# AndrewSigorskih/fastq-dupaway

Measured on AMD Instinct MI355X. Metric: Mreads/s dedup, 150 bp SE FASTQ (device phase: sequences resident in HBM), higher is better.
Workload: dtype u8

## Files before the change

fastq-dupaway_amd/csrc/fqd_engine.hip:

```cpp
#include <hip/hip_runtime.h>

#include <algorithm>
#include <chrono>
#include <cstdio>
#include <cstdlib>
#include <cstring>
#include <string>
#include <vector>

#include "fqd_internal.hpp"
#include "fqd_kernels.hpp"
#include "fqd_table_geometry.hpp"

using namespace fqd;

namespace {

thread_local std::string g_create_error;

struct DevBuf {
    void*  p = nullptr;
    size_t cap = 0;
    template <class T> T* as() const { return static_cast<T*>(p); }
};
// ... 282 lines not shown
    uint64_t* err = e->d_state;
    if (c.staged) {
        const uint32_t per_tile = e->S == 2 ? c.R / 2 : c.R;
        const uint32_t grid = uint32_t(std::min<uint64_t>((n + per_tile - 1) / per_tile, uint64_t(e->n_cu) * blocks_per_cu));
        static const size_t extra_lds = [] { const char* v = std::getenv("FQD_ENC_EXTRA_LDS"); return v ? size_t(std::max(0, std::atoi(v))) : size_t(0); }();
        const size_t lds = size_t(c.tile0) + c.tile1 + extra_lds;
        const uint32_t rw = ks.W0 + ks.lead;
        const uint32_t magic = rw > 1 ? uint32_t(((1ull << 32) + rw - 1) / rw) : 0xFFFFFFFFu;
        if (e->S == 1) {
            static const bool wide_out = [] { const char* v = std::getenv("FQD_ENC_STREAMOUT"); return !(v && v[0] == '0'); }();
            const bool pow2_rows = wide_out && rw >= 2 && (rw & (rw - 1)) == 0 && (reinterpret_cast<uintptr_t>(ks.keys) & 15u) == 0;
            const uint32_t magic1 = (c.lds_out && pow2_rows) ? 0u : magic;
            auto launch = [&](auto kernel) {
                hipLaunchKernelGGL(kernel, dim3(grid), dim3(c.R), lds, stream, sv[0], n, first_idx, ks, hash_out, err, magic1, h1);
            };
            if (c.lds_out) launch(encode_staged_kernel<true>); else launch(encode_staged_kernel<false>);
        } else {
            const uint32_t split = ks.lead + seg_words(seg[0].uniform_len);
            static const bool wide_out = [] { const char* v = std::getenv("FQD_ENC_STREAMOUT"); return !(v && v[0] == '0'); }();
            const bool pow2_rows = wide_out && rw >= 2 && (rw & (rw - 1)) == 0 && (split & 1u) == 0 && (reinterpret_cast<uintptr_t>(ks.keys) & 15u) == 0;
            const uint32_t magic2 = (c.lds_out && pow2_rows) ? 0u : magic;
            auto launch = [&](auto kernel) {
                hipLaunchKernelGGL(kernel, dim3(grid), dim3(c.R), lds, stream,
                                   sv[0], sv[1], n, first_idx, ks, hash_out, err, c.tile0, magic2, h1);
            };
            if (c.lds_out) launch(encode_staged_pe_kernel<true>); else launch(encode_staged_pe_kernel<false>);
        }
    } else if (!(e->flags & FQD_FLAG_NO_STAGE) && sv[0].offsets && (e->S == 1 || sv[1].offsets)) {
        const uint32_t R = 128, span_cap = e->S == 2 ? 24u * 1024u : 48u * 1024u;
        const uint32_t grid = uint32_t(std::min<uint64_t>((n + R - 1) / R, uint64_t(e->n_cu) * blocks_per_cu));
        if (e->S == 1)
            hipLaunchKernelGGL(encode_span_kernel<1>, dim3(grid), dim3(R), span_cap, stream,
                               sv[0], sv[1], n, first_idx, ks, hash_out, err, span_cap, h1);
        else
            hipLaunchKernelGGL(encode_span_kernel<2>, dim3(grid), dim3(R), 2 * span_cap, stream,
                               sv[0], sv[1], n, first_idx, ks, hash_out, err, span_cap, h1);
    } else {
        const uint32_t grid = uint32_t(std::min<uint64_t>(grid_for(e, n), uint64_t(e->n_cu) * blocks_per_cu));
        if (e->S == 1)
            hipLaunchKernelGGL(encode_general_kernel<1>, dim3(grid), dim3(kBlock), 0, stream,
                               sv[0], sv[1], n, first_idx, ks, hash_out, err, h1);
        else
            hipLaunchKernelGGL(encode_general_kernel<2>, dim3(grid), dim3(kBlock), 0, stream,
                               sv[0], sv[1], n, first_idx, ks, hash_out, err, h1);
    }
    HIP_TRY(e, hipGetLastError());
    return FQD_OK;
}

int launch_insert(fqd_engine* e, const KeyStore& ks, const uint64_t* hashes, uint32_t hash_stride,
                  uint64_t n, uint64_t first_idx, uint8_t* keep, bool preset_keep = true, uint32_t blocks_per_cu = 8,
                  uint32_t* first = nullptr)
{
    if (e->table_stale) {
        Bracket br(e, K_OTHER, 0);
        HIP_TRY(e, hipMemsetAsync(e->table.p, 0xFF, e->slots * sizeof(uint64_t), e->stream));
        e->table_stale = false;
    }
    e->table_clear = false;
    if (preset_keep) {
        Bracket br(e, K_OTHER, 0);
        HIP_TRY(e, hipMemsetAsync(keep, 1, n, e->stream));
    }
    Bracket br(e, K_INSERT, n);
    const uint32_t grid = uint32_t(std::min<uint64_t>(grid_for(e, n), uint64_t(e->n_cu) * blocks_per_cu));
    hipLaunchKernelGGL(insert_kernel, dim3(grid), dim3(kBlock), 0, e->stream,
                       e->table.as<uint64_t>(), e->slots - 1, (1ull << e->seg_bits) - 1, ks, hashes, hash_stride, n,
                       Verdicts{keep, first, uint32_t(first_idx)}, e->tag_mask,
                       reinterpret_cast<unsigned long long*>(e->d_state + 1));
    HIP_TRY(e, hipGetLastError());
    return FQD_OK;
}

bool bulk_applies(const fqd_engine* e, uint64_t n)
{
    if (n < e->bulk_min || e->slots < (1ull << 13)) return false;
    const bool empty = e->n_records == 0;
    static const uint64_t ratio = [] { const char* v = std::getenv("FQD_BULK_RATIO"); const long x = v ? std::atol(v) : 12; return uint64_t(x > 0 ? x : 12); }();
    return empty || n * ratio >= e->slots;
}

struct BulkPlan {
    bool ok = false;
    BulkGeom g{0, 0, 0, 0, 0};
    uint32_t nd1 = 0, n_buckets = 0;
    uint32_t *hist1 = nullptr, *start1 = nullptr, *cursor1 = nullptr, *tile_start1 = nullptr;
    uint32_t *hist2 = nullptr, *start2 = nullptr, *cursor2 = nullptr;
    uint64_t *recA = nullptr, *recB = nullptr;
    uint8_t *digit2 = nullptr;
    uint32_t *heavy_count = nullptr, *heavy_list = nullptr;
};

int bulk_plan(fqd_engine* e, uint64_t n, BulkPlan& p)
{
    uint32_t t = 0; while ((1ull << t) < e->slots) ++t;
    const uint32_t nb_bits = t - e->seg_bits;
    p.ok = false;
    if (nb_bits > 17 || nb_bits == 0) return FQD_OK;
    p.g.slot_mask = e->slots - 1; p.g.seg_bits = e->seg_bits; p.g.tag_mask = e->tag_mask;
    fqdgeom::table_digits(t, e->seg_bits, p.g.bits1, p.g.bits2);
    p.nd1 = 1u << p.g.bits1; p.n_buckets = 1u << nb_bits;
    int rc;
    const size_t rec_bytes = ((n * sizeof(uint64_t)) + 255) & ~size_t(255);
    const size_t d2_bytes = p.g.bits2 ? ((n * sizeof(uint8_t)) + 255) & ~size_t(255) : 0;
    if ((rc = reserve(e, e->bulk_recs, rec_bytes * (p.g.bits2 ? 2 : 1) + d2_bytes))) return rc;
    const size_t meta_words = 1100 + 4 * size_t(p.n_buckets) + 16;
    if ((rc = reserve(e, e->bulk_meta, meta_words * sizeof(uint32_t)))) return rc;
    uint32_t* m = e->bulk_meta.as<uint32_t>();
    p.hist1 = m; p.start1 = m + 256; p.cursor1 = m + 520; p.tile_start1 = m + 780;
    p.hist2 = m + 1100; p.start2 = p.hist2 + p.n_buckets; p.cursor2 = p.start2 + p.n_buckets + 4;
    p.heavy_count = m + 1090;
    p.heavy_list = p.cursor2 + p.n_buckets + 4;
    p.recA = e->bulk_recs.as<uint64_t>();
    p.recB = reinterpret_cast<uint64_t*>(e->bulk_recs.as<char>() + rec_bytes);
    p.digit2 = p.g.bits2 ? reinterpret_cast<uint8_t*>(e->bulk_recs.as<char>() + 2 * rec_bytes) : nullptr;
    {
        Bracket br(e, K_OTHER, 0);
        HIP_TRY(e, hipMemsetAsync(m, 0, meta_words * sizeof(uint32_t), e->stream));
    }
    p.ok = true;
    return FQD_OK;
}

int launch_bulk_insert(fqd_engine* e, const KeyStore& ks, const uint64_t* hashes, uint32_t hash_stride,
                       uint64_t n, uint64_t first_idx, uint8_t* keep, const BulkPlan& p, bool hist1_done,
                       uint32_t* first = nullptr, bool last_batch = false)
{
    const Verdicts verdicts{keep, first, uint32_t(first_idx)};
    const BulkGeom g = p.g;
    const uint32_t nd1 = p.nd1, n_buckets = p.n_buckets;
    uint32_t *hist1 = p.hist1, *start1 = p.start1, *cursor1 = p.cursor1, *tile_start1 = p.tile_start1;
    uint32_t *hist2 = p.hist2, *start2 = p.start2, *cursor2 = p.cursor2;
    uint64_t *recA = p.recA, *recB = p.recB;
    const bool fresh = e->n_records == 0 || e->table_clear || e->table_stale;
    {
        Bracket br(e, K_OTHER, 0);
        HIP_TRY(e, hipMemsetAsync(keep, 1, n, e->stream));
    }
    const uint64_t* final_recs = recA; const uint32_t* bstart = start1;
    {
    Bracket part_br(e, K_PARTITION, n);
    uint32_t part_per_cu = 2u;
    if (const char* v = std::getenv("FQD_PART_BLOCKS_PER_CU")) part_per_cu = uint32_t(std::min(16, std::max(1, std::atoi(v))));
    const uint32_t part_grid = uint32_t(std::min<uint64_t>((n + kPartTile - 1) / kPartTile, uint64_t(e->n_cu) * part_per_cu));
    if (!hist1_done)
        hipLaunchKernelGGL(bulk_hist1_kernel, dim3(part_grid), dim3(kPartThreads), 0, e->stream, hashes, hash_stride, n, g, hist1);
    hipLaunchKernelGGL(bulk_scan256_kernel, dim3(1), dim3(320), 0, e->stream,
                       static_cast<const uint32_t*>(hist1), nd1, start1, cursor1, tile_start1);
    hipLaunchKernelGGL(bulk_scatter_kernel<1>, dim3(part_grid), dim3(kPartThreads), 0, e->stream,
                       hashes, hash_stride, uint32_t(first_idx), static_cast<const uint64_t*>(nullptr), n, g,
                       static_cast<const uint32_t*>(start1), static_cast<const uint32_t*>(tile_start1), cursor1, recA, g.bits2 > 8 ? static_cast<uint8_t*>(nullptr) : p.digit2);
    if (g.bits2) {
        const uint32_t grid2 = uint32_t(std::min<uint64_t>((n + kPartTile - 1) / kPartTile + nd1, uint64_t(e->n_cu) * part_per_cu));
        const uint32_t hgrid = uint32_t(std::min<uint64_t>((n + kPartTile - 1) / kPartTile + nd1, uint64_t(e->n_cu) * 2u));
        if (g.bits2 > 8)
            hipLaunchKernelGGL(bulk_hist2_kernel<true>, dim3(hgrid), dim3(kPartThreads), 0, e->stream,
                               static_cast<const uint8_t*>(nullptr), static_cast<const uint64_t*>(recA), g, static_cast<const uint32_t*>(start1),
                               static_cast<const uint32_t*>(tile_start1), hist2);
        else
            hipLaunchKernelGGL(bulk_hist2_kernel<false>, dim3(hgrid), dim3(kPartThreads), 0, e->stream,
                               static_cast<const uint8_t*>(p.digit2), static_cast<const uint64_t*>(nullptr), g, static_cast<const uint32_t*>(start1),
                               static_cast<const uint32_t*>(tile_start1), hist2);
        hipLaunchKernelGGL(bulk_scan_buckets_kernel, dim3(nd1), dim3(512), 0, e->stream,
                           static_cast<const uint32_t*>(hist2), g.bits2, static_cast<const uint32_t*>(start1), nd1, start2, cursor2);
        hipLaunchKernelGGL(bulk_scatter_kernel<2>, dim3(grid2), dim3(kPartThreads), 0, e->stream,
                           static_cast<const uint64_t*>(nullptr), 0u, 0u, static_cast<const uint64_t*>(recA), n, g,
                           static_cast<const uint32_t*>(start1), static_cast<const uint32_t*>(tile_start1), cursor2, recB,
                           static_cast<uint8_t*>(nullptr));
        final_recs = recB; bstart = start2;
    }
    }
    Bracket br(e, K_DEDUP, n);
    const size_t lds = ((size_t(1) << e->seg_bits) + kDedupChunk + 2) * sizeof(uint64_t);
    uint32_t dthreads = 512;
    if (const char* v = std::getenv("FQD_DEDUP_THREADS")) dthreads = uint32_t(std::min(1024, std::max(64, std::atoi(v))));
    const uint32_t dgrid = std::min<uint32_t>(n_buckets, uint32_t(e->n_cu) * uint32_t(std::max<size_t>(1, (160 * 1024) / lds)));
    unsigned long long* counters = reinterpret_cast<unsigned long long*>(e->d_state + 1);
    uint32_t heavy_above = 4u << e->seg_bits;
    if (const char* v = std::getenv("FQD_HEAVY_ABOVE")) heavy_above = uint32_t(std::max(0, std::atoi(v)));
    static const bool force_write_back = [] { const char* v = std::getenv("FQD_FINAL_WRITE_BACK"); return v && v[0] == '1'; }();
    const uint32_t write_back = (last_batch && !force_write_back) ? 0u : 1u;
    auto launch_dedup = [&](auto kernel) -> int {
        if (lds > 64 * 1024) HIP_TRY(e, hipFuncSetAttribute(reinterpret_cast<const void*>(kernel), hipFuncAttributeMaxDynamicSharedMemorySize, int(lds)));
        hipLaunchKernelGGL(kernel, dim3(dgrid), dim3(dthreads), lds, e->stream,
                           final_recs, bstart, n_buckets, e->table.as<uint64_t>(), e->seg_bits, g.seg_bits + g.bits2, ks, verdicts, counters,
                           heavy_above, p.heavy_count, p.heavy_list, write_back);
        return FQD_OK;
    };
    int drc;
    int vl = 0;
    if (!ks.koff && ks.lead == 0 && ks.stride == ks.W0 && (ks.W0 & 1u) == 0) vl = ks.W0 <= 8 ? 4 : (ks.W0 <= 16 ? 8 : 0);
    if (const char* v = std::getenv("FQD_DEDUP_VL")) { if (std::atoi(v) == 0) vl = 0; }
    if (ks.koff)      drc = fresh ? launch_dedup(bucket_dedup_kernel<true, true, 0>) : launch_dedup(bucket_dedup_kernel<false, true, 0>);
    else if (vl == 4) drc = fresh ? launch_dedup(bucket_dedup_kernel<true, false, 4>) : launch_dedup(bucket_dedup_kernel<false, false, 4>);
    else if (vl == 8) drc = fresh ? launch_dedup(bucket_dedup_kernel<true, false, 8>) : launch_dedup(bucket_dedup_kernel<false, false, 8>);
    else              drc = fresh ? launch_dedup(bucket_dedup_kernel<true, false, 0>) : launch_dedup(bucket_dedup_kernel<false, false, 0>);
    if (drc) return drc;
    hipLaunchKernelGGL(heavy_bucket_insert_kernel, dim3(grid_for(e, n)), dim3(kBlock), 0, e->stream,
                       final_recs, bstart, g, e->table.as<uint64_t>(), ks, verdicts, counters,
                       static_cast<const uint32_t*>(p.heavy_count), static_cast<const uint32_t*>(p.heavy_list));
    HIP_TRY(e, hipGetLastError());
    e->table_clear = false; e->table_stale = !write_back;
    return FQD_OK;
}

int check_state(fqd_engine* e)
{
    HIP_TRY(e, hipMemcpyAsync(e->h_state, e->d_state, 5 * sizeof(uint64_t), hipMemcpyDeviceToHost, e->stream));
    HIP_TRY(e, hipStreamSynchronize(e->stream));
    if (e->flags & FQD_FLAG_PROFILE) drain_profile(e);
    if (e->h_state[2] != 0)
        return e->fail(FQD_ERR_HIP, "internal: hash set overflowed its table");
    if (e->h_state[4] != 0)
        return e->fail(FQD_ERR_ARG, "fqd_encode_padded: a read is longer than the key width the caller set (max_len0 / max_len1)");
    if (e->h_state[0] != kNoError) {
        const uint64_t w = e->h_state[0];
        e->has_bad = true;
        e->bad_record = w >> 32; e->bad_seg = uint32_t((w >> 31) & 1u);
        e->bad_pos = uint32_t((w >> 8) & 0x7FFFFFu); e->bad_byte = uint8_t(w & 0xFFu);
        char buf[160];
        std::snprintf(buf, sizeof buf, "unknown character in DNA sequence: byte 0x%02x at record %llu, mate %u, position %u",
                      unsigned(e->bad_byte), static_cast<unsigned long long>(e->bad_record), e->bad_seg + 1, e->bad_pos);
        return e->fail(FQD_ERR_BAD_BASE, buf);
    }
    return FQD_OK;
}

bool seg_is_uniform(const fqd_reads& r) { return r.offsets == nullptr && r.lengths == nullptr; }

}

FQD_HIDDEN hipStream_t fqd_internal_stream(fqd_engine* e) { return e->stream; }
FQD_HIDDEN int fqd_internal_device(fqd_engine* e) { return e->device; }
FQD_HIDDEN int fqd_internal_segments(fqd_engine* e) { return e->S; }
FQD_HIDDEN int fqd_internal_fail(fqd_engine* e, int code, const char* msg) { return e->fail(code, msg); }
FQD_HIDDEN uint64_t* fqd_internal_state(fqd_engine* e) { return e->d_state; }
FQD_HIDDEN int fqd_internal_scratch(fqd_engine* e, int which, size_t bytes, void** out)
{
    DevBuf& b = which == 0 ? e->scan_scratch : e->part_scratch;
    const int rc = reserve(e, b, bytes);
    *out = b.p;
    return rc;
}

extern "C" {

int fqd_abi_version(void) { return FQD_ABI_VERSION; }

int fqd_device_count(int* count)
{
    if (!count) return FQD_ERR_ARG;
    int n = 0;
    if (hipGetDeviceCount(&n) != hipSuccess) { *count = 0; return FQD_ERR_NO_DEVICE; }
    *count = n;
    return FQD_OK;
}

uint32_t fqd_key_words(uint32_t len0, uint32_t len1) { return seg_words(len0) + seg_words(len1); }

const char* fqd_last_error(const fqd_engine* e) { return e ? e->last_error.c_str() : g_create_error.c_str(); }

int fqd_engine_create(const fqd_config* cfg, fqd_engine** out)
{
    if (!cfg || !out || (cfg->segments != 1 && cfg->segments != 2)) { g_create_error = "bad fqd_config"; return FQD_ERR_ARG; }
    *out = nullptr;
    int ndev = 0;
    if (hipGetDeviceCount(&ndev) != hipSuccess || ndev <= 0 || cfg->device < 0 || cfg->device >= ndev) {
        g_create_error = "no HIP device available for the dedup engine (this library has no CPU path)";
        return FQD_ERR_NO_DEVICE;
    }
    fqd_engine* e = new fqd_engine();
    e->device = cfg->device; e->S = cfg->segments; e->flags = cfg->flags;
    e->cap_hint_reads = cfg->capacity_reads; e->cap_hint_bases = cfg->capacity_bases;
    auto bail = [&](const char* what, hipError_t err) {
        g_create_error = std::string(what) + ": " + hipGetErrorString(err);
        (void)hipGetLastError();
        delete e; return FQD_ERR_HIP;
    };
    hipError_t err;
    if ((err = hipSetDevice(e->device)) != hipSuccess) return bail("hipSetDevice", err);
    hipDeviceProp_t prop;
    if ((err = hipGetDeviceProperties(&prop, e->device)) != hipSuccess) return bail("hipGetDeviceProperties", err);
    e->n_cu = prop.multiProcessorCount > 0 ? prop.multiProcessorCount : 256;
    if (cfg->stream) { e->stream = static_cast<hipStream_t>(cfg->stream); }
    else {
        if ((err = hipStreamCreateWithFlags(&e->stream, hipStreamNonBlocking)) != hipSuccess) return bail("hipStreamCreate", err);
        e->own_stream = true;
    }
    if ((err = hipStreamCreateWithFlags(&e->aux, hipStreamNonBlocking)) != hipSuccess) return bail("hipStreamCreate(aux)", err);
    if (const char* v = std::getenv("FQD_CHUNK_READS")) { const long long x = std::atoll(v); e->chunk_reads = x > 0 ? uint64_t(x) : ~0ull; }
    if (const char* v = std::getenv("FQD_BULK_MIN")) { const long long x = std::atoll(v); e->bulk_min = x >= 0 ? uint64_t(x) : ~0ull; }
    if (const char* v = std::getenv("FQD_ENC_BLOCKS_PER_CU")) e->enc_blocks_per_cu = uint32_t(std::max(1, std::atoi(v)));
    if (const char* v = std::getenv("FQD_INS_BLOCKS_PER_CU")) e->ins_blocks_per_cu = uint32_t(std::max(1, std::atoi(v)));
    if ((err = hipMalloc(reinterpret_cast<void**>(&e->d_state), 8 * sizeof(uint64_t))) != hipSuccess) return bail("hipMalloc(state)", err);
    if ((err = hipHostMalloc(reinterpret_cast<void**>(&e->h_state), 8 * sizeof(uint64_t), hipHostMallocDefault)) != hipSuccess)
        return bail("hipHostMalloc(state)", err);
    int rc = fqd_engine_reset(e);
    if (rc == FQD_OK && cfg->capacity_reads) rc = ensure_table(e, cfg->capacity_reads, true);
    if (rc == FQD_OK && cfg->capacity_bases) {
        const uint64_t words = cfg->capacity_bases * 3 / 64 + 2 * cfg->capacity_reads + 1024;
        rc = reserve(e, e->keys, words * sizeof(uint64_t));
    }
    if (rc != FQD_OK) { g_create_error = e->last_error; fqd_engine_destroy(e); return rc; }
    *out = e;
    return FQD_OK;
}

int fqd_engine_destroy(fqd_engine* e)
{
    if (!e) return FQD_OK;
    (void)hipSetDevice(e->device);
    if (e->stream) (void)hipStreamSynchronize(e->stream);
#ifdef FQD_STAMPS
    {
        unsigned long long t[8][16];
        if (hipMemcpyFromSymbol(t, HIP_SYMBOL(g_stamps), sizeof t) == hipSuccess) {
            static const char* names[4] = {"scatter1", "scatter2", "dedup", "encode"};
            for (int k = 0; k < 4; ++k) {
                unsigned long long tot = 0; for (int q = 0; q < 16; ++q) tot += t[k][q];
                if (!tot) continue;
                std::fprintf(stderr, "[stamps] {\"kernel\": \"%s\", \"total_wg_ms\": %.3f, \"phase_frac\": [", names[k], double(tot) * 1e-5);
                for (int q = 0; q < 12; ++q) std::fprintf(stderr, "%s%.3f", q ? ", " : "", double(t[k][q]) / double(tot));
                std::fprintf(stderr, "]}\n");
            }
            std::memset(t, 0, sizeof t);
            (void)hipMemcpyToSymbol(HIP_SYMBOL(g_stamps), t, sizeof t);
        }
    }
#endif
// ... 604 lines not shown
```

fastq-dupaway_amd/csrc/fqd_kernels.hpp:

```cpp
#pragma once
#include "fqd_device.hpp"

namespace fqd {

constexpr int kBlock = 256;

#ifdef FQD_STAMPS
__device__ unsigned long long g_stamps[8][16];
#define STAMP_DECL __shared__ unsigned long long st_acc_[16]; __shared__ unsigned long long st_last_; \
    if (threadIdx.x == 0) { for (int q_ = 0; q_ < 16; ++q_) st_acc_[q_] = 0; st_last_ = wall_clock64(); }
#define STAMP(i) do { if (threadIdx.x == 0) { const unsigned long long now_ = wall_clock64(); st_acc_[i] += now_ - st_last_; st_last_ = now_; } } while (0)
#define STAMP_FLUSH(kid) do { if (threadIdx.x == 0) for (int q_ = 0; q_ < 16; ++q_) if (st_acc_[q_]) atomicAdd(&g_stamps[kid][q_], st_acc_[q_]); } while (0)
#define STAMP_LOADS_IN() asm volatile("s_waitcnt vmcnt(0)" ::: "memory")
#else
#define STAMP_LOADS_IN() do { } while (0)
#define STAMP_DECL
#define STAMP(i) do { } while (0)
#define STAMP_FLUSH(kid) do { } while (0)
#endif

struct SegView {
    const uint8_t*  bases;
    const uint64_t* offsets;
    const uint32_t* lengths;
// ... 363 lines not shown
            if (hash_out) hash_out[i] = hh;
            if (h1.hist) atomicAdd(&lhist[bucket_of(hh, h1.g) >> h1.g.bits2], 1u);
        }
        if (live && diff) {
            uint32_t byte = 0;
            const uint8_t* gp = (mate ? s1.bases : s0.bases) + i * uint64_t(stride);
            const uint32_t pos = first_bad_base(gp, len, &byte);
            if (pos != 0xFFFFFFFFu)
                atomicMin(reinterpret_cast<unsigned long long*>(err),
                          static_cast<unsigned long long>(make_error(first_idx + i, mate, pos, byte)));
        }
        if (LDS_OUT) {
            const uint32_t wave = t >> 6, lane = t & 63u;
            const uint32_t wave_pairs = (np > wave * 32u) ? ((np - wave * 32u < 32u) ? np - wave * 32u : 32u) : 0u;
            uint64_t* __restrict__ gout = ks.keys + (first_idx + r0 + wave * 32u) * uint64_t(ks.stride);
            const uint32_t total = wave_pairs * row_words, split = ks.lead + W_0;
#ifndef FQD_OLD_STREAMOUT
            if (rw_magic == 0u) {
                const uint32_t half_shift = uint32_t(__ffs(int(row_words))) - 2u;
                u64x2* __restrict__ gout2 = reinterpret_cast<u64x2*>(gout);
                for (uint32_t y = lane; y < (total >> 1); y += 64u) {
                    const uint32_t rr = y >> half_shift, kk = (y - (rr << half_shift)) << 1;
                    const uint32_t m = kk >= split ? 1u : 0u;
                    const uint32_t pb = in_base[m] + __umul24(wave * 32u + rr, m ? s1.ustride : s0.ustride);
                    const uint64_t* row = lds64 + ((pb + 4u + 7u) >> 3) + (m ? kk - split : kk);
                    const u64x2 v = {row[0], row[1]};
                    __builtin_nontemporal_store(v, &gout2[y]);
                }
            } else
#endif
            for (uint32_t x = lane; x < total; x += 64u) {
                const uint32_t rr = __umulhi(x, rw_magic), kk = x - rr * row_words;
                const uint32_t m = kk >= split ? 1u : 0u;
                const uint32_t kw = m ? kk - split : kk;
                const uint32_t pb = in_base[m] + (wave * 32u + rr) * (m ? s1.ustride : s0.ustride);
                __builtin_nontemporal_store(lds64[((pb + 4u + 7u) >> 3) + kw], &gout[x]);
            }
        }
        __syncthreads();
    }
    if (h1.hist) hist1_flush(lhist, h1.hist);
}

__device__ __forceinline__ bool keys_equal(const KeyStore& ks, uint32_t a, uint32_t b)
{
    const uint64_t* __restrict__ p = ks.slot(a);
    const uint64_t* __restrict__ q = ks.slot(b);
    uint32_t W = ks.W0;
    if (ks.koff) {
        const uint64_t ha = p[0];
        if (ha != q[0]) return false;
        W = seg_words(uint32_t(ha)) + seg_words(uint32_t(ha >> 32));
        ++p; ++q;
    }
    uint32_t k = 0;
    for (; k + 8u <= W; k += 8u) {
        uint64_t x[8], y[8];
#pragma unroll
        for (int j = 0; j < 8; ++j) { x[j] = p[k + j]; y[j] = q[k + j]; }
        uint64_t d = 0;
#pragma unroll
        for (int j = 0; j < 8; ++j) d |= x[j] ^ y[j];
        if (d) return false;
    }
    uint64_t d = 0;
    for (; k < W; ++k) d |= p[k] ^ q[k];
    return d == 0;
}

__global__ __launch_bounds__(kBlock)
void insert_kernel(uint64_t* __restrict__ table, uint64_t slot_mask, uint64_t seg_mask, KeyStore ks,
                   const uint64_t* __restrict__ hashes, uint32_t hash_stride,
                   uint64_t n, Verdicts out, uint32_t tag_mask,
                   unsigned long long* __restrict__ counters )
{
    unsigned long long* tab = reinterpret_cast<unsigned long long*>(table);
    uint32_t dups = 0, lost = 0;
    for (uint64_t i = blockIdx.x * uint64_t(kBlock) + threadIdx.x; i < n; i += uint64_t(gridDim.x) * kBlock) {
        const uint64_t h = hashes[i * uint64_t(hash_stride)];
        if (h == kSkipHash) continue;
        const uint32_t idx = out.first_idx + uint32_t(i);
        const uint64_t tag = slot_tag(h, tag_mask);
        const unsigned long long mine = (tag << 32) | idx;
        uint64_t pos = h & slot_mask;
        bool placed = false;
        for (uint64_t probe = 0; probe <= seg_mask; ++probe) {
            unsigned long long old = __hip_atomic_load(&tab[pos], __ATOMIC_RELAXED, __HIP_MEMORY_SCOPE_AGENT);
            if (old == kEmptySlot) {
                old = atomicCAS(&tab[pos], kEmptySlot, mine);
                if (old == kEmptySlot) { placed = true; break; }
            }
            if ((old >> 32) == tag && keys_equal(ks, idx, uint32_t(old))) {
                uint32_t owner = uint32_t(old);
                if (owner > idx) owner = uint32_t(atomicMin(&tab[pos], mine));
                if (owner < idx) out.lose(idx, owner);
                else             out.lose(owner, idx);
                ++dups;
                placed = true;
                break;
            }
            pos = (pos & ~seg_mask) | ((pos + 1) & seg_mask);
        }
        if (!placed) ++lost;
    }
#pragma unroll
    for (int d = 32; d > 0; d >>= 1) { dups += __shfl_down(dups, d, 64); lost += __shfl_down(lost, d, 64); }
    if ((threadIdx.x & 63) == 0) {
        if (dups) atomicAdd(&counters[0], static_cast<unsigned long long>(dups));
        if (lost) atomicAdd(&counters[1], static_cast<unsigned long long>(lost));
    }
}

__global__ __launch_bounds__(kBlock)
void rehash_kernel(const uint64_t* __restrict__ old_table, uint64_t old_slots,
                   uint64_t* __restrict__ new_table, uint64_t new_mask, uint64_t new_seg_mask, KeyStore ks,
                   uint32_t len0, uint32_t len1, uint32_t paired, uint64_t hash_and,
                   uint32_t new_tag_mask, unsigned long long* __restrict__ counters )
{
    unsigned long long* tab = reinterpret_cast<unsigned long long*>(new_table);
    for (uint64_t s = blockIdx.x * uint64_t(kBlock) + threadIdx.x; s < old_slots; s += uint64_t(gridDim.x) * kBlock) {
        const uint64_t e = old_table[s];
        if (e == kEmptySlot) continue;
        const uint32_t idx = uint32_t(e);
        const uint64_t* p = ks.slot(idx);
        uint32_t l0 = len0, l1 = len1, W = ks.W0;
        if (ks.koff) { l0 = uint32_t(p[0]); l1 = uint32_t(p[0] >> 32); W = seg_words(l0) + seg_words(l1); ++p; }
        const bool opaque = !ks.koff && len1 == kOpaqueKeys;
        if (opaque) paired = 0;
        const uint32_t w0 = opaque ? W : seg_words(l0);
        uint64_t h = hash_begin(l0, 0);
        for (uint32_t k = 0; k < w0; ++k) h = hash_word(h, p[k]);
        if (paired) {
            uint64_t h1 = hash_begin(l1, 0);
            for (uint32_t k = w0; k < W; ++k) h1 = hash_word(h1, p[k]);
            h = hash_pair(h, h1);
        } else {
            h = hash_end(h);
        }
        h &= hash_and;
        const unsigned long long mine = (slot_tag(h, new_tag_mask) << 32) | idx;
        uint64_t pos = h & new_mask;
        uint64_t probe = 0;
        while (atomicCAS(&tab[pos], kEmptySlot, mine) != kEmptySlot) {
            if (++probe > new_seg_mask) { atomicAdd(&counters[1], 1ull); break; }
            pos = (pos & ~new_seg_mask) | ((pos + 1) & new_seg_mask);
        }
    }
}


constexpr int kPartThreads = 1024;
constexpr int kPartPer = 8;
constexpr int kPartTile = kPartThreads * kPartPer;

__global__ __launch_bounds__(kPartThreads)
void bulk_hist1_kernel(const uint64_t* __restrict__ hashes, uint32_t hash_stride, uint64_t n, BulkGeom g,
                       uint32_t* __restrict__ hist1)
{
    __shared__ uint32_t h[256];
    for (int k = threadIdx.x; k < 256; k += kPartThreads) h[k] = 0;
    __syncthreads();
    for (uint64_t i = blockIdx.x * uint64_t(kPartThreads) + threadIdx.x; i < n; i += uint64_t(gridDim.x) * kPartThreads) {
        const uint64_t v = hashes[i * uint64_t(hash_stride)];
        if (v != kSkipHash) atomicAdd(&h[bucket_of(v, g) >> g.bits2], 1u);
    }
    __syncthreads();
    for (int k = threadIdx.x; k < 256; k += kPartThreads) if (h[k]) atomicAdd(&hist1[k], h[k]);
}

__global__ void bulk_scan256_kernel(const uint32_t* __restrict__ count, uint32_t nd, uint32_t* __restrict__ start,
                                    uint32_t* __restrict__ cursor, uint32_t* __restrict__ tile_start)
{
    __shared__ uint32_t a[257], t[257];
    const uint32_t d = threadIdx.x;
    if (d <= 256) {
        a[d] = d < nd ? count[d] : 0u;
        t[d] = d < nd ? (count[d] + kPartTile - 1) / kPartTile : 0u;
    }
    __syncthreads();
    if (d == 0) {
        uint32_t s = 0, ts = 0;
        for (uint32_t k = 0; k <= nd; ++k) { const uint32_t c = k < nd ? a[k] : 0, tc = k < nd ? t[k] : 0; a[k] = s; t[k] = ts; s += c; ts += tc; }
    }
    __syncthreads();
    if (d <= nd) { start[d] = a[d]; tile_start[d] = t[d]; if (d < nd) cursor[d] = a[d]; }
}

__device__ __forceinline__ uint32_t part_q(uint64_t hash, const BulkGeom& g)
{
    const uint32_t qshift = g.seg_bits + g.bits2;
    return (uint32_t(hash & g.slot_mask) & ((1u << qshift) - 1u)) | (uint32_t(slot_tag(hash, g.tag_mask)) << qshift);
}

template <int LEVEL>
__global__ __launch_bounds__(kPartThreads, 8)
void bulk_scatter_kernel(const uint64_t* __restrict__ hashes, uint32_t hash_stride, uint32_t first_idx,
                         const uint64_t* __restrict__ in, uint64_t n, BulkGeom g,
                         const uint32_t* __restrict__ start1, const uint32_t* __restrict__ tile_start1,
                         uint32_t* __restrict__ cursor, uint64_t* __restrict__ out,
                         uint8_t* __restrict__ digit2_out )
{
    __shared__ uint64_t stage[kPartTile];
    __shared__ uint8_t sdig[kPartTile];
    constexpr int kBins = (LEVEL == 1) ? 256 : 512;
    __shared__ uint32_t cnt[kBins], lstart[kBins], gbase[kBins];
    __shared__ uint32_t n_valid;
    const uint32_t nd1 = 1u << g.bits1, mask2 = (1u << g.bits2) - 1u;
    const uint64_t n_tiles = (LEVEL == 1) ? (n + kPartTile - 1) / kPartTile : tile_start1[nd1];
    STAMP_DECL
    for (uint64_t tile = blockIdx.x; tile < n_tiles; tile += gridDim.x) {
        STAMP(0);
        uint64_t lo, hi; uint32_t d1 = 0;
        if (LEVEL == 1) { lo = tile * kPartTile; hi = lo + kPartTile < n ? lo + kPartTile : n; }
        else {
            uint32_t a = 0, b = nd1;
            while (b - a > 1) { const uint32_t m = (a + b) >> 1; if (tile_start1[m] <= tile) a = m; else b = m; }
            d1 = a;
            lo = start1[d1] + (tile - tile_start1[d1]) * uint64_t(kPartTile);
            hi = lo + kPartTile < start1[d1 + 1] ? lo + kPartTile : start1[d1 + 1];
        }
        const uint32_t count = uint32_t(hi - lo);
        for (int k = threadIdx.x; k < kBins; k += kPartThreads) cnt[k] = 0;
        __syncthreads();
        STAMP(1);
        uint64_t rec[kPartPer]; uint32_t dig[kPartPer], rank[kPartPer];
#pragma unroll
        for (int k = 0; k < kPartPer; ++k) {
            const uint32_t r = threadIdx.x + k * kPartThreads;
            const uint64_t at = lo + (r < count ? r : count - 1u);
            rec[k] = (LEVEL == 1) ? hashes[at * uint64_t(hash_stride)] : in[at];
        }
        STAMP_LOADS_IN(); STAMP(10);
#pragma unroll
        for (int k = 0; k < kPartPer; ++k) {
            const uint32_t r = threadIdx.x + k * kPartThreads;
            dig[k] = 0xFFFFFFFFu;
            if (r < count && (LEVEL != 1 || rec[k] != kSkipHash)) {
                if (LEVEL == 1) {
                    const uint64_t h = rec[k];
                    rec[k] = (uint64_t(part_q(h, g)) << 32) | (first_idx + uint32_t(lo + r));
                    dig[k] = bucket_of(h, g) >> g.bits2;
                } else {
                    dig[k] = (uint32_t(rec[k] >> 32) >> g.seg_bits) & mask2;
                }
                rank[k] = atomicAdd(&cnt[dig[k]], 1u);
            }
        }
        STAMP(2);
        __syncthreads();
        STAMP(3);
        if (threadIdx.x < 64) {
            constexpr int kPer = kBins / 64;
            uint32_t c[kPer], s = 0;
#pragma unroll
            for (int k = 0; k < kPer; ++k) { c[k] = cnt[threadIdx.x * kPer + k]; s += c[k]; }
            uint32_t inc = s;
#pragma unroll
            for (int d = 1; d < 64; d <<= 1) { const uint32_t up = __shfl_up(inc, d, 64); if (int(threadIdx.x) >= d) inc += up; }
            uint32_t ex = inc - s;
#pragma unroll
            for (int k = 0; k < kPer; ++k) { lstart[threadIdx.x * kPer + k] = ex; ex += c[k]; }
            if (threadIdx.x == 63) n_valid = inc;
        }
        __syncthreads();
        STAMP(4);
        for (int k = threadIdx.x; k < kBins; k += kPartThreads)
            gbase[k] = cnt[k] ? atomicAdd(&cursor[(LEVEL == 1 ? 0u : (d1 << g.bits2)) + k], cnt[k]) : 0u;
        STAMP(5);
#pragma unroll
        for (int k = 0; k < kPartPer; ++k)
            if (dig[k] != 0xFFFFFFFFu) {
                const uint32_t at = lstart[dig[k]] + rank[k];
                stage[at] = rec[k];
                if (LEVEL == 1) sdig[at] = uint8_t(dig[k]);
            }
        STAMP(6);
        __syncthreads();
        STAMP(7);
        const uint32_t valid = n_valid;
#pragma unroll
        for (int k = 0; k < kPartPer; ++k) {
            const uint32_t r = threadIdx.x + k * kPartThreads;
            if (r < valid) {
                const uint64_t v = stage[r];
                const uint32_t d = (LEVEL == 1) ? uint32_t(sdig[r]) : ((uint32_t(v >> 32) >> g.seg_bits) & mask2);
                out[gbase[d] + (r - lstart[d])] = v;
                if (LEVEL == 1 && digit2_out) digit2_out[gbase[d] + (r - lstart[d])] = uint8_t((uint32_t(v >> 32) >> g.seg_bits) & mask2);
            }
        }
        STAMP(8);
        __syncthreads();
        STAMP(9);
    }
    STAMP_FLUSH(LEVEL - 1);
}

template <bool FROM_RECS>
__global__ __launch_bounds__(kPartThreads)
void bulk_hist2_kernel(const uint8_t* __restrict__ digit2_in, const uint64_t* __restrict__ recs, BulkGeom g, const uint32_t* __restrict__ start1,
                       const uint32_t* __restrict__ tile_start1, uint32_t* __restrict__ hist2)
{
    __shared__ uint32_t h[512];
    const uint32_t nd1 = 1u << g.bits1, nd2 = 1u << g.bits2;
    const uint64_t n_tiles = tile_start1[nd1];
    for (uint64_t tile = blockIdx.x; tile < n_tiles; tile += gridDim.x) {
        uint32_t a = 0, b = nd1;
        while (b - a > 1) { const uint32_t m = (a + b) >> 1; if (tile_start1[m] <= tile) a = m; else b = m; }
        const uint32_t d1 = a;
        const uint64_t lo = start1[d1] + (tile - tile_start1[d1]) * uint64_t(kPartTile);
        const uint64_t hi = lo + kPartTile < start1[d1 + 1] ? lo + kPartTile : start1[d1 + 1];
        for (uint32_t k = threadIdx.x; k < nd2; k += kPartThreads) h[k] = 0;
        __syncthreads();
        uint32_t dg[kPartPer];
#pragma unroll
        for (int k = 0; k < kPartPer; ++k) {
            const uint64_t r = lo + threadIdx.x + uint64_t(k) * kPartThreads, at = r < hi ? r : hi - 1;
            dg[k] = FROM_RECS ? (uint32_t(recs[at] >> 32) >> g.seg_bits) : uint32_t(digit2_in[at]);
        }
#pragma unroll
        for (int k = 0; k < kPartPer; ++k)
            if (lo + threadIdx.x + uint64_t(k) * kPartThreads < hi) atomicAdd(&h[dg[k] & (nd2 - 1u)], 1u);
        __syncthreads();
        for (uint32_t k = threadIdx.x; k < nd2; k += kPartThreads) if (h[k]) atomicAdd(&hist2[(d1 << g.bits2) + k], h[k]);
        __syncthreads();
    }
}

__global__ __launch_bounds__(512)
void bulk_scan_buckets_kernel(const uint32_t* __restrict__ count, uint32_t bits2, const uint32_t* __restrict__ start1,
                              uint32_t nd1, uint32_t* __restrict__ start, uint32_t* __restrict__ cursor)
{
    __shared__ uint32_t wave_tot[8];
    const uint32_t nd2 = 1u << bits2, d1 = blockIdx.x, t = threadIdx.x;
    const uint32_t c = t < nd2 ? count[(d1 << bits2) + t] : 0u;
    uint32_t inc = c;
#pragma unroll
    for (int d = 1; d < 64; d <<= 1) { const uint32_t up = __shfl_up(inc, d, 64); if (int(t & 63u) >= d) inc += up; }
    if ((t & 63u) == 63u) wave_tot[t >> 6] = inc;
    __syncthreads();
    uint32_t before = start1[d1];
    for (uint32_t w = 0; w < (t >> 6); ++w) before += wave_tot[w];
    if (t < nd2) { start[(d1 << bits2) + t] = before + inc - c; cursor[(d1 << bits2) + t] = before + inc - c; }
    if (d1 == nd1 - 1u && t == 0) start[nd1 << bits2] = start1[nd1];
}

constexpr uint32_t kDedupChunk = 1536;
constexpr uint32_t kDedupRecords = 3 * kDedupChunk;
constexpr uint32_t kDedupFly = 4;
#ifndef FQD_DEDUP_LOADS
#define FQD_DEDUP_LOADS 6
#endif
#ifndef FQD_DEDUP_EARLY
#define FQD_DEDUP_EARLY 1
#endif
constexpr uint32_t kDedupLoads = FQD_DEDUP_LOADS;

template <bool FRESH, bool RAGGED, int VL>
__global__ __launch_bounds__(1024)
void bucket_dedup_kernel(const uint64_t* __restrict__ recs, const uint32_t* __restrict__ bstart, uint32_t n_buckets,
                         uint64_t* __restrict__ table, uint32_t seg_bits, uint32_t qshift, KeyStore ks, Verdicts out,
                         unsigned long long* __restrict__ counters,
                         uint32_t heavy_above, uint32_t* __restrict__ heavy_count, uint32_t* __restrict__ heavy_list,
                         uint32_t write_back)
{
    extern __shared__ __attribute__((aligned(16))) unsigned long long seg[];
    const uint32_t seg_slots = 1u << seg_bits, seg_mask = seg_slots - 1u;
    unsigned long long* queue = seg + seg_slots;
    uint32_t* qn = reinterpret_cast<uint32_t*>(queue + kDedupChunk);
    uint32_t dups = 0, lost = 0;

    auto walk = [&](uint32_t idx, uint32_t tag32, uint32_t pos, bool verify_inline) {
        const uint64_t tag = tag32;
        const unsigned long long mine = (tag << 32) | idx;
        for (uint32_t probe = 0; probe < seg_slots; ++probe) {
            const unsigned long long old = atomicCAS(&seg[pos], kEmptySlot, mine);
            if (old == kEmptySlot) return;
            if ((old >> 32) == tag) {
                if (!verify_inline) {
                    const uint32_t at = atomicAdd(&qn[0], 1u);
                    if (at < kDedupChunk) { queue[at] = (uint64_t((tag32 << seg_bits) | pos) << 32) | idx; return; }
                }
                if (keys_equal(ks, idx, uint32_t(old))) {
                    uint32_t owner = uint32_t(old);
                    if (owner > idx) owner = uint32_t(atomicMin(&seg[pos], mine));
                    if (owner < idx) out.lose(idx, owner);
                    else             out.lose(owner, idx);
                    ++dups;
                    return;
                }
            }
            pos = (pos + 1u) & seg_mask;
        }
        ++lost;
    };

    STAMP_DECL
    for (uint32_t b = blockIdx.x; b < n_buckets; b += gridDim.x) {
        STAMP(0);
        unsigned long long* gseg = reinterpret_cast<unsigned long long*>(table) + uint64_t(b) * seg_slots;
        const uint32_t lo = bstart[b], hi = bstart[b + 1];
        if (!FRESH && lo == hi) continue;
        if (hi - lo > heavy_above) {
            if (FRESH) for (uint32_t k = threadIdx.x; k < seg_slots; k += blockDim.x) gseg[k] = kEmptySlot;
            if (threadIdx.x == 0) heavy_list[atomicAdd(heavy_count, 1u)] = b;
            continue;
        }
        uint64_t v0[kDedupLoads];
        {
            const uint32_t first_n = hi - lo < kDedupRecords ? hi - lo : kDedupRecords;
#pragma unroll
            for (uint32_t u = 0; u < kDedupLoads; ++u) { const uint32_t c = threadIdx.x + u * blockDim.x; v0[u] = (FQD_DEDUP_EARLY && first_n) ? recs[lo + (c < first_n ? c : first_n - 1u)] : 0ull; }
        }
        {
            ulonglong2* seg2 = reinterpret_cast<ulonglong2*>(seg);
            const ulonglong2* gseg2 = reinterpret_cast<const ulonglong2*>(gseg);
            const uint32_t n2 = seg_slots >> 1;
            if (FRESH) {
                for (uint32_t k = threadIdx.x; k < n2; k += blockDim.x) seg2[k] = ulonglong2{kEmptySlot, kEmptySlot};
            } else {
                for (uint32_t k0 = threadIdx.x; k0 < n2; k0 += 4u * blockDim.x) {
                    ulonglong2 v[4];
#pragma unroll
                    for (uint32_t u = 0; u < 4u; ++u) { const uint32_t k = k0 + u * blockDim.x; v[u] = gseg2[k < n2 ? k : n2 - 1u]; }
#pragma unroll
                    for (uint32_t u = 0; u < 4u; ++u) { const uint32_t k = k0 + u * blockDim.x; if (k < n2) seg2[k] = v[u]; }
                }
            }
        }
        for (uint32_t chunk_lo = lo; chunk_lo < hi; chunk_lo += kDedupRecords) {
            const uint32_t chunk_n = hi - chunk_lo < kDedupRecords ? hi - chunk_lo : kDedupRecords;
            if (threadIdx.x == 0) { qn[0] = 0; qn[1] = 0; }
            __syncthreads();
            STAMP(1);
            for (uint32_t c0 = threadIdx.x; c0 < chunk_n; c0 += kDedupLoads * blockDim.x) {
                uint64_t v[kDedupLoads];
                if (FQD_DEDUP_EARLY && chunk_lo == lo && c0 == threadIdx.x) {
#pragma unroll
                    for (uint32_t u = 0; u < kDedupLoads; ++u) v[u] = v0[u];
                } else {
#pragma unroll
                    for (uint32_t u = 0; u < kDedupLoads; ++u) { const uint32_t c = c0 + u * blockDim.x; v[u] = recs[chunk_lo + (c < chunk_n ? c : chunk_n - 1u)]; }
                }
                STAMP_LOADS_IN(); STAMP(9);
#pragma unroll
                for (uint32_t u = 0; u < kDedupLoads; ++u) {
                    if (c0 + u * blockDim.x < chunk_n) {
                        const uint32_t q = uint32_t(v[u] >> 32);
                        walk(uint32_t(v[u]), q >> qshift, q & seg_mask, false);
                    }
                }
            }
            STAMP(2);
            __syncthreads();
            STAMP(3);
            const uint32_t n_cand = qn[0] < kDedupChunk ? qn[0] : kDedupChunk;
            constexpr uint32_t kFly = RAGGED ? 3u : (VL == 4 ? 6u : kDedupFly);
            constexpr uint32_t kLanes = VL ? uint32_t(VL) : 8u;
            const uint32_t grp = threadIdx.x / kLanes, n_grp = blockDim.x / kLanes, sub = threadIdx.x % kLanes;
            for (uint32_t q0 = grp; q0 < n_cand; q0 += n_grp * kFly) {
                uint32_t pos[kFly], idx[kFly], seen[kFly], tag[kFly];
                uint64_t diff[kFly];
                bool live[kFly];
                uint64_t wa[kFly][2], wb[kFly][2];
#pragma unroll
                for (uint32_t u = 0; u < kFly; ++u) {
                    const uint32_t q = q0 + u * n_grp;
                    live[u] = q < n_cand;
                    diff[u] = 0; pos[u] = 0; idx[u] = 0; seen[u] = 0; tag[u] = 0;
                    wa[u][0] = wa[u][1] = wb[u][0] = wb[u][1] = 0;
                    if (live[u]) {
                        const unsigned long long ent = queue[q];
                        idx[u] = uint32_t(ent); pos[u] = uint32_t(ent >> 32) & seg_mask; tag[u] = uint32_t(ent >> 32) >> seg_bits;
                        seen[u] = uint32_t(seg[pos[u]]);
                    }
                    if (!RAGGED && VL) {
                        const ulonglong2* __restrict__ pa = reinterpret_cast<const ulonglong2*>(ks.keys + idx[u] * uint64_t(ks.stride));
                        const ulonglong2* __restrict__ pb = reinterpret_cast<const ulonglong2*>(ks.keys + seen[u] * uint64_t(ks.stride));
// ... 654 lines not shown
```

Measured before the change: 14660.

## Stretch hist2 over multi-tile spans with vector loads; wave-parallel scan256

Adds a second-level histogram kernel in which each block walks runs of up to eight tiles. Contiguous tiles from the same first-level digit are merged, and byte digits are read as 16-byte vector loads. This cuts per-tile block overhead, the binary searches and global atomic flushes, and it shrinks the hist2 grid. The single-thread serial 256-entry prefix scan is also replaced by a one-wave shuffle scan, and an env override is added to cap the dedup grid. The new hist2 path has more complex boundary handling, and fewer blocks may reduce parallelism for small inputs.

```diff
diff --git a/fastq-dupaway_amd/csrc/fqd_engine.hip b/fastq-dupaway_amd/csrc/fqd_engine.hip
--- a/fastq-dupaway_amd/csrc/fqd_engine.hip
+++ b/fastq-dupaway_amd/csrc/fqd_engine.hip
@@ -458,15 +458,14 @@
                        static_cast<const uint32_t*>(start1), static_cast<const uint32_t*>(tile_start1), cursor1, recA, g.bits2 > 8 ? static_cast<uint8_t*>(nullptr) : p.digit2);
     if (g.bits2) {
         const uint32_t grid2 = uint32_t(std::min<uint64_t>((n + kPartTile - 1) / kPartTile + nd1, uint64_t(e->n_cu) * part_per_cu));
-        const uint32_t hgrid = uint32_t(std::min<uint64_t>((n + kPartTile - 1) / kPartTile + nd1, uint64_t(e->n_cu) * 2u));
-        if (g.bits2 > 8)
-            hipLaunchKernelGGL(bulk_hist2_kernel<true>, dim3(hgrid), dim3(kPartThreads), 0, e->stream,
-                               static_cast<const uint8_t*>(nullptr), static_cast<const uint64_t*>(recA), g, static_cast<const uint32_t*>(start1),
-                               static_cast<const uint32_t*>(tile_start1), hist2);
-        else
-            hipLaunchKernelGGL(bulk_hist2_kernel<false>, dim3(hgrid), dim3(kPartThreads), 0, e->stream,
-                               static_cast<const uint8_t*>(p.digit2), static_cast<const uint64_t*>(nullptr), g, static_cast<const uint32_t*>(start1),
-                               static_cast<const uint32_t*>(tile_start1), hist2);
+        const uint64_t htiles = (n + kPartTile - 1) / kPartTile + nd1, hwork = FQD_HIST2_STRETCH ? (htiles + kHistTiles - 1) / kHistTiles : htiles;
+        const uint32_t hgrid = uint32_t(std::min<uint64_t>(hwork, uint64_t(e->n_cu) * 2u));
+        auto launch_hist2 = [&](auto kernel, const uint8_t* digits, const uint64_t* records) {
+            hipLaunchKernelGGL(kernel, dim3(hgrid), dim3(kPartThreads), 0, e->stream, digits, records, g,
+                               static_cast<const uint32_t*>(start1), static_cast<const uint32_t*>(tile_start1), hist2);
+        };
+        if (g.bits2 > 8) launch_hist2(FQD_HIST2_STRETCH ? bulk_hist2_stretch_kernel<true> : bulk_hist2_kernel<true>, nullptr, recA);
+        else             launch_hist2(FQD_HIST2_STRETCH ? bulk_hist2_stretch_kernel<false> : bulk_hist2_kernel<false>, p.digit2, nullptr);
         hipLaunchKernelGGL(bulk_scan_buckets_kernel, dim3(nd1), dim3(512), 0, e->stream,
                            static_cast<const uint32_t*>(hist2), g.bits2, static_cast<const uint32_t*>(start1), nd1, start2, cursor2);
         hipLaunchKernelGGL(bulk_scatter_kernel<2>, dim3(grid2), dim3(kPartThreads), 0, e->stream,
@@ -480,7 +479,8 @@
     const size_t lds = ((size_t(1) << e->seg_bits) + kDedupChunk + 2) * sizeof(uint64_t);
     uint32_t dthreads = 512;
     if (const char* v = std::getenv("FQD_DEDUP_THREADS")) dthreads = uint32_t(std::min(1024, std::max(64, std::atoi(v))));
-    const uint32_t dgrid = std::min<uint32_t>(n_buckets, uint32_t(e->n_cu) * uint32_t(std::max<size_t>(1, (160 * 1024) / lds)));
+    uint32_t dgrid = std::min<uint32_t>(n_buckets, uint32_t(e->n_cu) * uint32_t(std::max<size_t>(1, (160 * 1024) / lds)));
+    if (const char* v = std::getenv("FQD_DEDUP_GRID")) dgrid = std::min<uint32_t>(dgrid, uint32_t(std::max(1, std::atoi(v))));
     unsigned long long* counters = reinterpret_cast<unsigned long long*>(e->d_state + 1);
     uint32_t heavy_above = 4u << e->seg_bits;
     if (const char* v = std::getenv("FQD_HEAVY_ABOVE")) heavy_above = uint32_t(std::max(0, std::atoi(v)));
diff --git a/fastq-dupaway_amd/csrc/fqd_kernels.hpp b/fastq-dupaway_amd/csrc/fqd_kernels.hpp
--- a/fastq-dupaway_amd/csrc/fqd_kernels.hpp
+++ b/fastq-dupaway_amd/csrc/fqd_kernels.hpp
@@ -539,6 +539,13 @@
 constexpr int kPartThreads = 1024;
 constexpr int kPartPer = 8;
 constexpr int kPartTile = kPartThreads * kPartPer;
+#ifndef FQD_SCAN256_WAVE
+#define FQD_SCAN256_WAVE 1
+#endif
+#ifndef FQD_HIST2_STRETCH
+#define FQD_HIST2_STRETCH 1
+#endif
+constexpr uint32_t kHistTiles = 8;
 
 __global__ __launch_bounds__(kPartThreads)
 void bulk_hist1_kernel(const uint64_t* __restrict__ hashes, uint32_t hash_stride, uint64_t n, BulkGeom g,
@@ -565,7 +572,23 @@
         t[d] = d < nd ? (count[d] + kPartTile - 1) / kPartTile : 0u;
     }
     __syncthreads();
-    if (d == 0) {
+    if (FQD_SCAN256_WAVE) {
+        if (d < 64) {
+            uint32_t c[4], tc[4], s = 0, ts = 0;
+#pragma unroll
+            for (uint32_t k = 0; k < 4; ++k) { const uint32_t i = d * 4 + k; c[k] = i < nd ? a[i] : 0u; tc[k] = i < nd ? t[i] : 0u; s += c[k]; ts += tc[k]; }
+            uint32_t inc = s, tinc = ts;
+#pragma unroll
+            for (int w = 1; w < 64; w <<= 1) {
+                const uint32_t up = __shfl_up(inc, w, 64), tup = __shfl_up(tinc, w, 64);
+                if (int(d) >= w) { inc += up; tinc += tup; }
+            }
+            uint32_t ex = inc - s, tex = tinc - ts;
+#pragma unroll
+            for (uint32_t k = 0; k < 4; ++k) { const uint32_t i = d * 4 + k; a[i] = ex; t[i] = tex; ex += c[k]; tex += tc[k]; }
+            if (d == 63) { a[256] = inc; t[256] = tinc; }
+        }
+    } else if (d == 0) {
         uint32_t s = 0, ts = 0;
         for (uint32_t k = 0; k <= nd; ++k) { const uint32_t c = k < nd ? a[k] : 0, tc = k < nd ? t[k] : 0; a[k] = s; t[k] = ts; s += c; ts += tc; }
     }
@@ -710,6 +733,75 @@
         __syncthreads();
         for (uint32_t k = threadIdx.x; k < nd2; k += kPartThreads) if (h[k]) atomicAdd(&hist2[(d1 << g.bits2) + k], h[k]);
         __syncthreads();
+    }
+}
+
+template <bool FROM_RECS>
+__global__ __launch_bounds__(kPartThreads)
+void bulk_hist2_stretch_kernel(const uint8_t* __restrict__ digit2_in, const uint64_t* __restrict__ recs, BulkGeom g, const uint32_t* __restrict__ start1,
+                               const uint32_t* __restrict__ tile_start1, uint32_t* __restrict__ hist2)
+{
+    __shared__ uint32_t h[512];
+    constexpr uint32_t kVecLoads = 4;
+    const uint32_t nd1 = 1u << g.bits1, nd2 = 1u << g.bits2, m2 = nd2 - 1u;
+    const uint64_t n_tiles = tile_start1[nd1];
+    for (uint32_t k = threadIdx.x; k < nd2; k += kPartThreads) h[k] = 0;
+    __syncthreads();
+    for (uint64_t t0 = uint64_t(blockIdx.x) * kHistTiles; t0 < n_tiles; t0 += uint64_t(gridDim.x) * kHistTiles) {
+        const uint64_t t1 = t0 + kHistTiles < n_tiles ? t0 + kHistTiles : n_tiles;
+        uint32_t a = 0, b = nd1;
+        while (b - a > 1) { const uint32_t m = (a + b) >> 1; if (tile_start1[m] <= t0) a = m; else b = m; }
+        uint32_t d1 = a;
+        for (uint64_t t = t0; t < t1; ++d1) {
+            while (tile_start1[d1 + 1] <= t) ++d1;
+            const uint64_t ts = tile_start1[d1], te = tile_start1[d1 + 1] < t1 ? uint64_t(tile_start1[d1 + 1]) : t1;
+            const uint64_t lo = start1[d1] + (t - ts) * kPartTile, end = start1[d1 + 1];
+            const uint64_t hi = start1[d1] + (te - ts) * kPartTile < end ? start1[d1] + (te - ts) * kPartTile : end;
+            if (FROM_RECS) {
+                for (uint64_t r0 = lo; r0 < hi; r0 += kPartTile) {
+                    uint32_t dg[kPartPer];
+#pragma unroll
+                    for (int k = 0; k < kPartPer; ++k) {
+                        const uint64_t r = r0 + threadIdx.x + uint64_t(k) * kPartThreads, at = r < hi ? r : hi - 1;
+                        dg[k] = uint32_t(recs[at] >> 32) >> g.seg_bits;
+                    }
+#pragma unroll
+                    for (int k = 0; k < kPartPer; ++k)
+                        if (r0 + threadIdx.x + uint64_t(k) * kPartThreads < hi) atomicAdd(&h[dg[k] & m2], 1u);
+                }
+            } else {
+                const uint64_t to_unit = (16u - uint32_t(reinterpret_cast<uintptr_t>(digit2_in + lo) & 15u)) & 15u;
+                const uint64_t a0 = lo + to_unit < hi ? lo + to_unit : hi;
+                const uint64_t a1 = a0 + ((hi - a0) & ~uint64_t(15));
+                if (threadIdx.x < uint32_t(a0 - lo)) atomicAdd(&h[digit2_in[lo + threadIdx.x] & m2], 1u);
+                if (threadIdx.x < uint32_t(hi - a1)) atomicAdd(&h[digit2_in[a1 + threadIdx.x] & m2], 1u);
+                const uint4* __restrict__ units = reinterpret_cast<const uint4*>(digit2_in + a0);
+                const uint32_t n_units = uint32_t((a1 - a0) >> 4);
+                for (uint32_t u0 = 0; u0 < n_units; u0 += kVecLoads * kPartThreads) {
+                    uint4 w[kVecLoads];
+#pragma unroll
+                    for (uint32_t u = 0; u < kVecLoads; ++u) { const uint32_t i = u0 + threadIdx.x + u * kPartThreads; w[u] = units[i < n_units ? i : n_units - 1u]; }
+#pragma unroll
+                    for (uint32_t u = 0; u < kVecLoads; ++u) {
+                        if (u0 + threadIdx.x + u * kPartThreads < n_units) {
+                            const uint32_t x[4] = {w[u].x, w[u].y, w[u].z, w[u].w};
+#pragma unroll
+                            for (int q = 0; q < 4; ++q) {
+                                atomicAdd(&h[x[q] & 0xFFu & m2], 1u); atomicAdd(&h[(x[q] >> 8) & 0xFFu & m2], 1u);
+                                atomicAdd(&h[(x[q] >> 16) & 0xFFu & m2], 1u); atomicAdd(&h[(x[q] >> 24) & m2], 1u);
+                            }
+                        }
+                    }
+                }
+            }
+            __syncthreads();
+            for (uint32_t k = threadIdx.x; k < nd2; k += kPartThreads) {
+                const uint32_t c = h[k];
+                if (c) { atomicAdd(&hist2[(d1 << g.bits2) + k], c); h[k] = 0; }
+            }
+            __syncthreads();
+            t = te;
+        }
     }
 }
 
```

New measurement: 14770, median of 6. Within noise of the previous version (+0.8%).
